# PreibischLab/multiview-simulation

Measured on AMD Instinct MI355X. Metric: simulated Mvoxel/s (views x input voxels / s), 512^3 volume x 8 views, higher is better.
Workload: dtype f32 (f64 attenuation/reductions/Poisson)

## Files before the change

### multiview-simulation_amd/build.py

```python
from __future__ import annotations

import os
import shutil
import subprocess
import sys

HERE = os.path.dirname(os.path.abspath(__file__))
CSRC = os.path.join(HERE, "csrc")
LIB = os.path.join(HERE, "libmvsim.so")
SOURCES = ["api.cpp", "api_view.cpp", "api_host.cpp", "api_sims.cpp", "comm.cpp", "kernels.hip", "extract.hip", "fftconv.hip", "fft_kernels.hip", "rotate_fft.hip", "stencil.hip", "phantom.hip", "beads.hip", "aberrations.hip", "procedural.hip"]
HEADERS = ["common.h", "api_internal.h", "host_pool.h", "jrandom.h", "extract_plan.h", "poisson_dev.h", "fft_dev.h", "../../include/mvsim.h"]
ROCM = os.environ.get("ROCM_PATH", "/opt/rocm")


def _hipcc() -> str:
    for cand in (os.path.join(ROCM, "bin", "hipcc"), shutil.which("hipcc")):
        if cand and os.path.exists(cand):
            return cand
    raise RuntimeError("hipcc not found (ROCm toolchain required to build libmvsim.so)")


def sources():
    return [os.path.join(CSRC, s) for s in SOURCES if os.path.exists(os.path.join(CSRC, s))]


def source_sha() -> str:
    import hashlib
    h = hashlib.sha256()
    files = sorted(sources() + [os.path.normpath(os.path.join(CSRC, x)) for x in HEADERS])
    for f in files:
        h.update(os.path.basename(f).encode() + b"\0")
        with open(f, "rb") as fh:
            h.update(fh.read())
    return h.hexdigest()[:16]


def _common_flags():
    return [
        "--offload-arch=gfx950", "-O3", "-std=c++17", "-fPIC", "-ffp-contract=off", "-fno-fast-math",
        *os.environ.get("MVSIM_EXTRA_CFLAGS", "").split(),
        "-Wall", "-Wno-unused-result", "-I" + os.path.join(ROCM, "include"),
    ]


def is_current() -> bool:
    if not os.path.exists(LIB) or not os.path.exists(LIB + ".flags"):
        return False
    with open(LIB + ".flags") as fh:
        if fh.read() != " ".join(_common_flags()):
            return False
    t = os.path.getmtime(LIB)
    deps = sources() + [os.path.normpath(os.path.join(CSRC, h)) for h in HEADERS] + [os.path.abspath(__file__)]
    return all(os.path.getmtime(d) <= t for d in deps if os.path.exists(d))


def build(force: bool = False, verbose: bool = False) -> str:
    if not force and is_current():
        return LIB
    hipcc = _hipcc()
    objs = []
    os.makedirs(os.path.join(HERE, "build"), exist_ok=True)
    common = _common_flags()
    flags_id = " ".join(common)
    hdr_time = max(os.path.getmtime(os.path.normpath(os.path.join(CSRC, h))) for h in HEADERS)
    hdr_time = max(hdr_time, os.path.getmtime(os.path.abspath(__file__)))
    procs = []
    for src in sources():
        obj = os.path.join(HERE, "build", os.path.basename(src) + ".o")
        objs.append(obj)
        stamp = obj + ".flags"
        fresh = (not force and os.path.exists(obj) and os.path.exists(stamp) and open(stamp).read() == flags_id
                 and os.path.getmtime(obj) >= max(os.path.getmtime(src), hdr_time))
        if fresh:
            continue
        cmd = [hipcc, "-x", "hip", "-c", src, "-o", obj] + common
        if verbose:
            print(" ".join(cmd), file=sys.stderr)
        procs.append((src, stamp, subprocess.Popen(cmd, stdout=subprocess.PIPE, stderr=subprocess.STDOUT, text=True)))
    failed = False
    for src, stamp, p in procs:
        out, _ = p.communicate()
        if p.returncode != 0:
            failed = True
            if os.path.exists(stamp):
                os.remove(stamp)
            sys.stderr.write(f"--- {src} ---\n{out}\n")
        else:
            with open(stamp, "w") as fh:
                fh.write(flags_id)
            if verbose and out.strip():
                sys.stderr.write(out)
    if failed:
        raise RuntimeError("hipcc failed")
    link = [hipcc, "-shared", "-fPIC", "--offload-arch=gfx950", "-o", LIB] + objs + [
# ... 13 lines not shown
```

### multiview-simulation_amd/csrc/api.cpp

```cpp
#include "api_internal.h"

#include <cstdlib>
#include <mutex>
#include <thread>

namespace mvsim {

static thread_local char g_err[512] = "";

void set_error(const char* fmt, ...)
{
    va_list ap;
    va_start(ap, fmt);
    vsnprintf(g_err, sizeof(g_err), fmt, ap);
    va_end(ap);
}

int parse_option(Options& o, const char* name, const char* value)
{
    if (!name || !value) return MVSIM_EINVAL;
    const std::string n(name), v(value);
    auto word = [&](std::initializer_list<std::pair<const char*, int>> words, auto* dst) {
        for (const auto& w : words)
            if (v == w.first) { *dst = w.second; return MVSIM_OK; }
        return MVSIM_EINVAL;
    };
    auto flag = [&](bool* dst) { return word({{"1", 1}, {"on", 1}, {"true", 1}, {"0", 0}, {"off", 0}, {"false", 0}}, dst); };
    auto number = [&](size_t digits, long long lo, long long hi, auto* dst, int when_auto = -1) {
        if (when_auto >= 0 && v == "auto") { *dst = when_auto; return MVSIM_OK; }
        if (v.empty() || v.size() > digits || v.find_first_not_of("0123456789") != std::string::npos) return MVSIM_EINVAL;
        const long long k = atoll(v.c_str());
        if (k < lo || k > hi) return MVSIM_EINVAL;
        *dst = k;
        return MVSIM_OK;
    };
    if (n == "fft_zpass") return word({{"auto", 0}, {"direct", 1}, {"fft", 2}, {"inline", 3}}, &o.zpass);
    if (n == "fft_backend") return word({{"custom", 0}, {"auto", 0}, {"rocfft", 1}}, &o.rocfft);
    if (n == "fused_rotate") return word({{"1", 1}, {"on", 1}, {"lds", 1}, {"0", 0}, {"off", 0}, {"2", 2}, {"lane", 2}, {"3", 3}, {"auto", 3}}, &o.fused_rotate);
    if (n == "poisson_queue") return word({{"1", 1}, {"on", 1}, {"0", 0}, {"off", 0}}, &o.poisson_queue);
    if (n == "poisson_queue_share") return number(2, 1, 16, &o.poisson_queue_share, 0);
    if (n == "attenuate") return word({{"serial", 0}, {"scan", 1}}, &o.attenuate_scan);
    if (n == "early_sum") return flag(&o.early_sum);
    if (n == "zconv_strided") return flag(&o.zconv_strided);
    if (n == "exp") return number(2, 0, 15, &o.exp);
    if (n == "beads_pair_cap") return number(10, 1024, 1LL << 31, &o.beads_pair_cap);
    if (n == "reject_batch") return number(7, 1, 1LL << 20, &o.reject_batch, 0);
    if (n == "fuse_tail") return flag(&o.fuse_tail);
    if (n == "psf_overlap") return flag(&o.psf_overlap);
    if (n == "fused_fftx") return word({{"auto", 2}, {"1", 1}, {"on", 1}, {"0", 0}, {"off", 0}}, &o.fused_fftx);
    if (n == "tail_overlap") return word({{"0", 0}, {"off", 0}, {"1", 1}, {"on", 1}, {"own", 1}, {"2", 2}, {"any", 2}}, &o.tail_overlap);
    if (n == "acq_transfer") return word({{"auto", 1}, {"u16", 1}, {"f32", 0}}, &o.acq_u16);
    if (n == "host_threads") return number(3, 1, 256, &o.host_threads, 0);
    if (n == "view_batch") return word({{"auto", 2}, {"1", 1}, {"on", 1}, {"0", 0}, {"off", 0}}, &o.view_batch);
    if (n == "view_lanes") return number(2, 1, MVSIM_MAX_VIEWS, &o.view_lanes, 0);
    if (n == "graph") { bool g = false; const int rc = flag(&g); o.graph = g ? 1 : 0; return rc; }
    if (n == "broadcast") {
        int how = 0;
        if (word({{"scatter_allgather", 0}, {"auto", 0}, {"ring", 1}, {"peer_copy", 2}, {"pipelined", 3}}, &how) != MVSIM_OK) return MVSIM_EINVAL;
        o.bcast_ring = how == 1; o.bcast_peer_copy = how == 2; o.bcast_pipelined = how == 3;
        return MVSIM_OK;
    }
    if (n == "skip_empty") return flag(&o.skip_empty);
    if (n == "fft_pad") {
        long long a = 0, b = 0, c = 0;
        if (v == "auto" || v.empty()) { o.fft_pad[0] = o.fft_pad[1] = o.fft_pad[2] = 0; return MVSIM_OK; }
        if (sscanf(v.c_str(), "%lld,%lld,%lld", &a, &b, &c) != 3 || a < 0 || b < 0 || c < 0) return MVSIM_EINVAL;
        o.fft_pad[0] = a; o.fft_pad[1] = b; o.fft_pad[2] = c;
        return MVSIM_OK;
    }
    return MVSIM_EINVAL;
}

const Options& env_options()
{
    static Options o;
    static std::once_flag once;
    std::call_once(once, [] {
        if (const char* e = getenv("MVSIM_FFT_ZPASS")) (void)parse_option(o, "fft_zpass", e);
        if (const char* e = getenv("MVSIM_FFT_BACKEND")) (void)parse_option(o, "fft_backend", e);
        if (const char* e = getenv("MVSIM_FFT_PAD")) (void)parse_option(o, "fft_pad", e);
        if (getenv("MVSIM_NO_FUSED_ROTATE")) o.fused_rotate = 0;
        if (getenv("MVSIM_POISSON_NOQUEUE")) o.poisson_queue = 0;
        if (getenv("MVSIM_NO_EARLY_SUM")) o.early_sum = false;
        if (getenv("MVSIM_NO_FUSE_TAIL")) o.fuse_tail = false;
        if (const char* e = getenv("MVSIM_GRAPH")) (void)parse_option(o, "graph", e);
        if (const char* e = getenv("MVSIM_BROADCAST")) (void)parse_option(o, "broadcast", e);
        if (const char* e = getenv("MVSIM_OPTIONS")) {
            std::string all(e);
            size_t pos = 0;
            while (pos < all.size()) {
                size_t end = all.find(';', pos);
                if (end == std::string::npos) end = all.size();
                const std::string kv = all.substr(pos, end - pos);
                const size_t eq = kv.find('=');
                if (eq != std::string::npos) (void)parse_option(o, kv.substr(0, eq).c_str(), kv.substr(eq + 1).c_str());
                pos = end + 1;
            }
        }
    });
    return o;
}

int ensure_lds_attr(mvsim_ctx* ctx, const void* kernel, size_t bytes)
{
    if (bytes <= 64 * 1024) return MVSIM_OK;
    if (bytes > 160 * 1024) { set_error("kernel needs %zu bytes of LDS (> 160 KiB)", bytes); return MVSIM_EINVAL; }
    if (ctx->lds_attr_set.count(kernel)) return MVSIM_OK;
    MVSIM_HIP(hipFuncSetAttribute(kernel, hipFuncAttributeMaxDynamicSharedMemorySize, 160 * 1024));
    ctx->lds_attr_set.insert(kernel);
    return MVSIM_OK;
}

int DevBuf::reserve(size_t need)
{
    if (need <= bytes) return MVSIM_OK;
    if (epoch) *epoch += 1;
    if (p) { (void)hipFree(p); p = nullptr; bytes = 0; }
    hipError_t e = hipMalloc(&p, need);
    if (e != hipSuccess) {
        p = nullptr;
        set_error("hipMalloc(%zu bytes) failed: %s", need, hipGetErrorString(e));
        return MVSIM_ENOMEM;
    }
    bytes = need;
    return MVSIM_OK;
}

void DevBuf::release()
{
    if (p && epoch) *epoch += 1;
    if (p) (void)hipFree(p);
    p = nullptr;
// ... 721 lines not shown
```

### multiview-simulation_amd/csrc/fft_dev.h

```cpp
#pragma once

#include "common.h"

namespace mvsim {
namespace fft {

__device__ __forceinline__ float2 cadd(float2 a, float2 b) { return make_float2(a.x + b.x, a.y + b.y); }
__device__ __forceinline__ float2 csub(float2 a, float2 b) { return make_float2(a.x - b.x, a.y - b.y); }
__device__ __forceinline__ float2 cmul(float2 a, float2 b)
{
    return make_float2(fmaf(a.x, b.x, -a.y * b.y), fmaf(a.x, b.y, a.y * b.x));
}
__device__ __forceinline__ float2 cconj(float2 a) { return make_float2(a.x, -a.y); }
__device__ __forceinline__ float2 mul_mi(float2 a) { return make_float2(a.y, -a.x); }

template <int R> __device__ __forceinline__ void dft(float2* u);

template <> __device__ __forceinline__ void dft<2>(float2* u)
{
    const float2 a = u[0], b = u[1];
    u[0] = cadd(a, b);
    u[1] = csub(a, b);
}

// ... 284 lines not shown
    return -1;
}

struct SrcMap {
    DimMap x, y, z;
    int    enum_y;
};

struct __attribute__((packed, aligned(8))) Pair16 {
    float a, b, c, d;
};

#ifdef MVSIM_DEV_SIZES
#define MVSIM_FFT_SIZES(X) X(280, 7, 5, 8) X(560, 7, 8, 10)
#else
#define MVSIM_FFT_SIZES(X) \
    X(16, 4, 4)            \
    X(18, 9, 2)            \
    X(20, 5, 4)            \
    X(24, 3, 8)            \
    X(32, 4, 8)            \
    X(36, 9, 4)            \
    X(40, 5, 8)            \
    X(48, 3, 4, 4)         \
    X(56, 7, 8)            \
    X(64, 8, 8)            \
    X(72, 9, 8)            \
    X(80, 5, 4, 4)         \
    X(96, 3, 8, 4)         \
    X(112, 7, 4, 4)        \
    X(128, 4, 8, 4)        \
    X(140, 7, 5, 4)        \
    X(144, 9, 4, 4)        \
    X(160, 5, 8, 4)        \
    X(180, 9, 5, 4)        \
    X(192, 3, 8, 8)        \
    X(224, 7, 8, 4)        \
    X(256, 4, 8, 8)        \
    X(280, 7, 5, 8)        \
    X(288, 9, 8, 4)        \
    X(320, 5, 8, 8)        \
    X(350, 7, 10, 5)       \
    X(360, 9, 5, 8)        \
    X(384, 3, 8, 4, 4)     \
    X(448, 7, 8, 8)        \
    X(512, 8, 8, 8)        \
    X(540, 9, 5, 4, 3)     \
    X(560, 7, 8, 10)       \
    X(576, 9, 8, 8)        \
    X(640, 5, 8, 4, 4)     \
    X(720, 9, 8, 10)       \
    X(768, 3, 8, 8, 4)     \
    X(896, 7, 8, 4, 4)     \
    X(1024, 4, 8, 8, 4)    \
    X(1080, 9, 8, 5, 3)    \
    X(1120, 7, 8, 5, 4)    \
    X(1152, 9, 8, 4, 4)    \
    X(1280, 5, 8, 8, 4)    \
    X(1440, 9, 8, 5, 4)    \
    X(1536, 3, 8, 8, 8)    \
    X(1792, 7, 8, 8, 4)    \
    X(2048, 8, 8, 8, 4)    \
    X(2160, 10, 8, 9, 3)   \
    X(2240, 7, 8, 8, 5)
#endif

struct RotFftArgs {
    const float* in;
    float*       rot_out;
    float*       att_out;
    float2*      dst;
    const float2* twg;
    const float2* twx;
    int nx, ny, nz, steps;
    int z_first, nzl;
    int hxp, py;
    int halo_r, halo_l;
    Affine a;
    double delta;
    int*   plane_nz;
};

constexpr bool rot_fftx_len_ok(int len) { return len >= 72 && len <= 576; }
int  launch_rot_fftx(mvsim_ctx* ctx, int M, const RotFftArgs& a, bool write_out);

}
}
```

### multiview-simulation_amd/csrc/fft_kernels.hip

```cpp
#include "common.h"
#include "fft_dev.h"
#include "poisson_dev.h"

#include <algorithm>
#include <cmath>
#include <cstdlib>
#include <cstring>

namespace mvsim {
static int ensure_twiddles(mvsim_ctx* ctx, int L, int kind, const float2** out);
namespace fft {

enum Mode { FWD = 0, INV = 1, CONV = 2, CONVZ = 3 };

struct LinesArgs {
    const float2* src;
    float2*       dst;
    const float2* spec;
    const float2* tw;
    long long     src_es, src_outer, dst_es, dst_outer, spec_es, spec_outer;
    DimMap        lmap;
    int           gap_lo, gap_hi;
    int           outer_skip_lo, outer_skip_len;
    int           store_limit;
// ... 1533 lines not shown

size_t fused_tail_queue_bytes(const int64_t dim[3], const int64_t kdim[3], int inc, bool con_wanted, const Options& opt)
{
    ExtractPlan fp{};
    return fused_tail_geometry(dim, kdim, inc, con_wanted, opt, &fp) ? fp.layout.total_bytes : 0;
}

void custom_fft_release(mvsim_ctx* ctx)
{
    for (auto& kv : ctx->twiddles) (void)hipFree(kv.second);
    ctx->twiddles.clear();
    for (auto& kv : ctx->box_weights) (void)hipFree(kv.second);
    ctx->box_weights.clear();
    ctx->partials_z.release();
    ctx->cfft_f.release();
    ctx->cfft_g.release();
    ctx->cfft_g1.release();
    ctx->cfft_g2.release();
}

bool custom_fft_geometry(const int64_t dim[3], const int64_t kdim[3], int64_t g[5], const Options& opt)
{
    ConvPlan pl;
    if (!conv_plan(dim, kdim, opt, &pl)) return false;
    g[0] = pl.px; g[1] = pl.py; g[2] = pl.zdirect ? pl.n[2] : pl.pz; g[3] = pl.hxp; g[4] = pl.zdirect ? 1 : 0;
    return true;
}

bool custom_fft_batchable(const mvsim_ctx* ctx, const int64_t dim[3], const int64_t kdim[3])
{
    const Options& o = ctx->opt;
    ConvPlan pl;
    return conv_plan(dim, kdim, o, &pl) && pl.early && !o.fuse_tail && o.zpass != 3 && !pl.zinline_auto && pl.ymirror;
}

int rotate_attenuate_fftx(mvsim_ctx* ctx, const float* gt, float* rot_or_null, float* att_or_null, const int64_t dim[3],
                          const int64_t kdim[3], const Affine& inv, double delta, bool* done, const int** plane_nz, int z_first, int nzl)
{
    using namespace fft;
    *done = false;
    if (plane_nz) *plane_nz = nullptr;
    if (ctx->opt.fused_fftx == 0) return MVSIM_OK;
    const bool x_identity = inv.m[0] == 1.0 && inv.m[1] == 0.0 && inv.m[2] == 0.0 && inv.m[3] == 0.0 &&
                            inv.m[4] == 0.0 && inv.m[8] == 0.0;
    if (!x_identity) return MVSIM_OK;
    ConvPlan pl;
    if (!conv_plan(dim, kdim, ctx->opt, &pl)) return MVSIM_OK;
    const int nx = pl.n[0], ny = pl.n[1], nz = pl.n[2], kx = pl.k[0];
    if (nzl < 0) { z_first = 0; nzl = nz; }
    if (z_first < 0 || nzl < 1 || z_first + nzl > nz) return MVSIM_OK;
    if (!pl.ymirror || nx > 1024 || nx < 64 || kx > nx || nx > ny) return MVSIM_OK;
    const int px = pl.px, py = pl.py, M = pl.M, hxp = pl.hxp;
    if (!rot_fftx_len_ok(M)) return MVSIM_OK;
    if (ctx->opt.fused_fftx == 2 && (int64_t)nx * nzl < 131072) return MVSIM_OK;
    const size_t cbytes = pl.spectrum_bytes(nzl, 0, 0, 1);
    MVSIM_TRY(ctx->cfft_f.reserve(cbytes));
    MVSIM_TRY(ctx->cfft_g.reserve(cbytes));
    const float2 *tw_m, *tw_px;
    MVSIM_TRY(ensure_twiddles(ctx, M, 0, &tw_m));
    MVSIM_TRY(ensure_twiddles(ctx, px, 1, &tw_px));
    RotFftArgs a{};
    a.in = gt; a.rot_out = rot_or_null; a.att_out = att_or_null; a.dst = ctx->cfft_f.as<float2>();
    a.twg = tw_m; a.twx = tw_px;
    a.nx = nx; a.ny = ny; a.nz = nz; a.steps = nx;
    a.z_first = z_first; a.nzl = nzl;
    a.hxp = hxp; a.py = py;
    a.halo_r = kx / 2; a.halo_l = kx - 1 - kx / 2;
    a.a = inv; a.delta = delta;
    bool want_flags = plane_nz && ctx->opt.skip_empty && nzl == nz;
    if (want_flags) {
        if (!ctx->empty_hint) {
            MVSIM_HIP(hipHostMalloc(reinterpret_cast<void**>(&ctx->empty_hint), 4 * sizeof(int), hipHostMallocDefault));
            ctx->empty_hint[0] = -1; ctx->empty_hint[1] = -1; ctx->empty_hint[2] = 0; ctx->empty_hint[3] = 0;
        }
        const int hint = *reinterpret_cast<volatile int*>(ctx->empty_hint);
        if (hint == 0 && ctx->views_since_flags < 15) { want_flags = false; ctx->views_since_flags += 1; }
        else ctx->views_since_flags = 0;
    }
    if (want_flags) {
        MVSIM_TRY(ctx->plane_flags.reserve((size_t)(3 * nz + 1024) * sizeof(int)));
        a.plane_nz = ctx->plane_flags.as<int>();
        *plane_nz = a.plane_nz;
    }
    MVSIM_TRY(launch_rot_fftx(ctx, M, a, rot_or_null != nullptr || att_or_null != nullptr));
    *done = true;
    return MVSIM_OK;
}

namespace fft {
struct ConvRun {
    const ConvPlan& pl;
    SlabRange slab;
    const LenEntry* xlen;
    bool is_slab;
    long long plane;
    int V, zstride;
    int nzp;
    int nk;
    int zs_chunk, zs_frows;
    size_t zs_lds;
    bool zinline;
    long long corr_n;
    float corr_min, corr_target;
    const float2 *tw_m, *tw_px, *tw_py, *tw_pz;
    float2 *F, *G, *G1, *G2;
    double* scal;
    const int *pnz, *pnz_dil;
    const unsigned int* pnz_bits;
};

static int psf_passes(mvsim_ctx* ctx, const ConvRun& r, const float* psf)
{
    const ConvPlan& pl = r.pl;
    const int kx = pl.k[0], ky = pl.k[1], kz = pl.k[2], hxp = pl.hxp, V = r.V;
    SrcMap m{};
    m.x = DimMap{kx, pl.px, kx - kx / 2, kx / 2, 1, kx / 2};
    m.y = DimMap{ky, ky, ky, 0, 1, 0};
    m.z = DimMap{kz * V, kz * V, kz * V, 0, 1, 0};
    MVSIM_TRY(r.xlen->r2c(ctx, psf, m, r.G1, r.tw_m, r.tw_px, hxp, (long long)ky * kz * V));
    LinesArgs a{};
    a.src = r.G1; a.dst = r.G2; a.spec = nullptr; a.tw = r.tw_py;
    a.src_es = hxp; a.src_outer = (long long)hxp * ky;
    a.dst_es = hxp; a.dst_outer = r.plane;
    if (pl.zdirect) { a.dst_outer = (long long)ZB * hxp; a.dst_blk = (long long)kz * V * ZB * hxp; }
    a.lmap = DimMap{ky, pl.py, ky - ky / 2, ky / 2, 1, ky / 2};
    MVSIM_TRY(launch_lines(ctx, pl.py, FWD, true, a, hxp / pl.tile_y, kz * V));
    if (pl.zdirect) return MVSIM_OK;
    LinesArgs c{};
    c.src = r.G2; c.dst = r.G; c.spec = nullptr; c.tw = r.tw_pz;
    c.src_es = r.plane; c.src_outer = hxp;
    c.dst_es = r.plane; c.dst_outer = hxp;
    c.lmap = DimMap{kz, pl.pz, kz - kz / 2, kz / 2, 1, kz / 2};
    c.dst_tile_major = 1;
    return launch_lines(ctx, pl.pz, FWD, true, c, hxp / pl.tile_z, pl.py);
}

static int psf_spectrum(mvsim_ctx* ctx, const ConvRun& r, const float* psf)
{
    hipStream_t s = ctx->stream;
    const bool side = ctx->opt.psf_overlap && (int64_t)r.pl.n[0] * r.pl.n[1] * r.pl.n[2] >= (int64_t)1 << 24;
    ctx->psf_on_side = side;
    if (side) {
        if (!ctx->side_stream) {
            MVSIM_HIP(hipStreamCreateWithFlags(&ctx->side_stream, hipStreamNonBlocking));
            MVSIM_HIP(hipEventCreateWithFlags(&ctx->ev_fork, hipEventDisableTiming));
            MVSIM_HIP(hipEventCreateWithFlags(&ctx->ev_join, hipEventDisableTiming));
        }
        MVSIM_HIP(hipEventRecord(ctx->ev_fork, s));
        MVSIM_HIP(hipStreamWaitEvent(ctx->side_stream, ctx->ev_fork, 0));
        ctx->stream = ctx->side_stream;
    }
    ev_begin(ctx, ST_PSF);
    const int rc = psf_passes(ctx, r, psf);
    ev_end(ctx, ST_PSF);
    if (side) {
        ctx->stream = s;
        MVSIM_HIP(hipEventRecord(ctx->ev_join, ctx->side_stream));
    }
    return rc;
}

static int pass_a(mvsim_ctx* ctx, const ConvRun& r, const float* img)
{
    const ConvPlan& pl = r.pl;
    const int planes = r.slab.nz_in * r.V;
    SrcMap m{};
    DimMap* dm[3] = {&m.x, &m.y, &m.z};
// ... 288 lines not shown
```

### multiview-simulation_amd/csrc/rotate_fft.hip

```cpp
#include "common.h"
#include "fft_dev.h"

#include <type_traits>

namespace mvsim {
namespace fft {

struct __attribute__((aligned(16))) RowGeoF {
    double    w00, w10, w11, w01;
    long long off00;
    int       kind;
    int       pad;
};
constexpr int geo_chunk_f(int G) { return G == 1 ? 512 : 128; }
constexpr int UF = 8;
#ifndef MVSIM_ROTFFT_PREFETCH
#define MVSIM_ROTFFT_PREFETCH 0
#endif

template <class PLAN, bool WRITE_OUT, int G>
__global__ __launch_bounds__(1024) void k_rotate_attenuate_fftx(RotFftArgs p)
{
    constexpr int M = PLAN::len, LP = M + 1, U = UF, GEO_CHUNK_F = geo_chunk_f(G);
    extern __shared__ __align__(16) float2 lds[];
    float2* rowbuf = lds;
    float2* tw = lds + 2 * G * U * LP;
    float2* twx_l = tw + M + (M & 1);
    RowGeoF* geo = reinterpret_cast<RowGeoF*>(twx_l + (M + 1) + ((M + 1) & 1));
    int* bclass = reinterpret_cast<int*>(geo + GEO_CHUNK_F);
    unsigned int* wmask = reinterpret_cast<unsigned int*>(bclass + GEO_CHUNK_F / U);
    const int nx = p.nx, ny = p.ny, nz = p.nz, steps = p.steps;
    const int x = threadIdx.x;
    const int lane = x & 63, wave = __builtin_amdgcn_readfirstlane(x >> 6), nwaves = (int)blockDim.x >> 6;
    const int slab = (gridDim.x + 7) / 8;
    const int hs = slab / 2, jb = (int)(blockIdx.x / 8u), kb = (int)(blockIdx.x % 8u);
    const int zl = (hs > 0 && slab == 2 * hs) ? ((jb < hs) ? kb * hs + jb : (int)gridDim.x / 2 + kb * hs + (jb - hs))
                                              : kb * slab + jb;
    if (zl >= p.nzl) return;
    const int z = p.z_first + zl;
    const bool active = x < nx;
    const long long row = (long long)nx;
    const long long plane = row * ny;
    const long long out_plane = plane * zl;
    const double l2 = (double)z;
    const char* __restrict__ in_b = reinterpret_cast<const char*>(p.in);
    const long long row_b = row * 4, plane_b = plane * 4;
    const unsigned xoff = (unsigned)(active ? x : nx - 1) * 4u;
    const Affine& a = p.a;
    const double delta = p.delta;
    const int Px = 2 * M;
    const int pos_r = (active && x >= nx - 1 - p.halo_r && x <= nx - 2) ? 2 * nx - 2 - x : -1;
    const int pos_l = (active && x >= 1 && x <= p.halo_l) ? Px - x : -1;
    const int gap_lo = nx + p.halo_r, gap_len = Px - p.halo_l - gap_lo;
    for (int i = x; i < M; i += (int)blockDim.x) tw[i] = p.twg[i];
    for (int i = x; i <= M; i += (int)blockDim.x) twx_l[i] = p.twx[i];

    auto transform_store = [&](float2* wbuf, int y) {
        PLAN::template run<1>(wbuf, tw, lane);
        float2* __restrict__ drow = p.dst + ((long long)zl * p.py + y) * p.hxp;
        constexpr int HQ = M / 4;
#pragma unroll 1
        for (int q = lane; q < HQ; q += 64) {
            float2 lo[2], hi[2];
#pragma unroll
            for (int h = 0; h < 2; ++h) {
                const int k = 2 * q + h;
                const float2 zk = wbuf[k];
                const float2 zm = cconj(wbuf[k == 0 ? 0 : M - k]);
                const float2 sm = cadd(zk, zm), d = csub(zk, zm);
                const float2 wd = cmul(twx_l[k], d);
                const float2 t = make_float2(wd.y, -wd.x);
                lo[h] = cadd(sm, t);
                hi[h] = cconj(csub(sm, t));
            }
            *reinterpret_cast<float4*>(drow + 2 * q) = make_float4(lo[0].x, lo[0].y, lo[1].x, lo[1].y);
            *reinterpret_cast<Pair16*>(drow + M - 2 * q - 1) = Pair16{hi[1].x, hi[1].y, hi[0].x, hi[0].y};
        }
        const int nmid = M - 4 * HQ + 1;
        const int ntail = nmid + (p.hxp - M - 1);
        for (int u = lane; u < ntail; u += 64) {
            if (u < nmid) {
                const int k = 2 * HQ + u;
                const float2 zk = wbuf[k == M ? 0 : k];
                const float2 zm = cconj(wbuf[k == 0 ? 0 : M - k]);
// ... 159 lines not shown
                            const float a10 = (active && t10) ? p00[row + x] : 0.f;
                            const float a11 = (active && t11) ? p00[row + plane + x] : 0.f;
                            const float a01 = (active && t01) ? p00[plane + x] : 0.f;
                            r = (float)((double)a00 * g->w00);
                            r += (float)((double)a10 * g->w10);
                            r += (float)((double)a11 * g->w11);
                            r += (float)((double)a01 * g->w01);
                            const double d = (double)r;
                            n = fmax(n - d * delta * n, 0.0);
                            val[u] = (float)(d * n);
                        }
                        if (WRITE_OUT && active) {
                            if (p.rot_out) p.rot_out[o + x] = r;
                            if (p.att_out) p.att_out[o + x] = val[u];
                        }
                    }
                }
            }
            {
                unsigned int rowmask = 0u;
#pragma unroll
                for (int u = 0; u < U; ++u)
                    if (__builtin_amdgcn_ballot_w64(active && (__float_as_uint(val[u]) << 1) != 0u) != 0ull) rowmask |= 1u << u;
                if (lane == 0) wmask[(buf * G + fill) * 16 + wave] = rowmask;
                plane_any |= rowmask;
            }
            float* __restrict__ rb = reinterpret_cast<float*>(rowbuf + ((size_t)buf * G + fill) * U * LP);
            ysub[fill] = y0;
            nsub[fill] = nrows;
            fill += 1;
#pragma unroll
            for (int u = 0; u < U; ++u) {
                float* __restrict__ rr = rb + (size_t)u * 2 * LP;
                if (active) rr[x] = val[u];
                if (pos_r >= 0) rr[pos_r] = val[u];
                if (pos_l >= 0) rr[pos_l] = val[u];
                for (int gpos = x; gpos < gap_len; gpos += (int)blockDim.x) rr[gap_lo + gpos] = 0.f;
            }
            have_pref = r0 + U < cnt && __builtin_amdgcn_readfirstlane(bclass[r0 / U + 1]) == 1;
            if (have_pref) issue_loads(r0 + U, std::integral_constant<int, 0>{}, std::integral_constant<int, UPRE>{});
            if (fill == G) flush_round();
        }
        if (fill > 0) flush_round();
    }
    if (p.plane_nz) {
        unsigned int* blk_any = wmask + 2 * G * 16;
        __syncthreads();
        if (x == 0) *blk_any = 0u;
        __syncthreads();
        if (lane == 0 && plane_any != 0u) atomicOr(blk_any, 1u);
        __syncthreads();
        if (x == 0) p.plane_nz[zl] = (int)*blk_any;
    }
    for (int yy = ny - 1 - steps; yy >= 0; --yy) {
        if (WRITE_OUT && active) {
            if (p.att_out) p.att_out[out_plane + (long long)yy * row + x] = 0.f;
            if (p.rot_out) {
                const double l1 = (double)yy;
                const double py = 0.0 * a.m[4] + l1 * a.m[5] + l2 * a.m[6] + a.m[7];
                const double pz = 0.0 * a.m[8] + l1 * a.m[9] + l2 * a.m[10] + a.m[11];
                const double fy = floor(py), fz = floor(pz);
                float o = 0.f;
                if (fy >= -1.0 && fz >= -1.0 && fy < (double)ny && fz < (double)nz) {
                    const int sy = (int)fy, sz = (int)fz;
                    const double w1 = py - fy, w2 = pz - fz;
                    const double w1n = 1.0 - w1, w2n = 1.0 - w2;
                    const double q00 = 1.0 * w1n * w2n, q10 = 1.0 * w1 * w2n, q11 = 1.0 * w1 * w2, q01 = 1.0 * w1n * w2;
                    const bool ya = sy >= 0, yb = sy + 1 < ny, za = sz >= 0, zb = sz + 1 < nz;
                    const float* __restrict__ pin = p.in + x;
                    const float a00 = (ya && za) ? pin[row * (sy + (long long)ny * sz)] : 0.f;
                    const float a10 = (yb && za) ? pin[row * (sy + 1 + (long long)ny * sz)] : 0.f;
                    const float a11 = (yb && zb) ? pin[row * (sy + 1 + (long long)ny * (sz + 1))] : 0.f;
                    const float a01 = (ya && zb) ? pin[row * (sy + (long long)ny * (sz + 1))] : 0.f;
                    o = (float)((double)a00 * q00); o += (float)((double)a10 * q10);
                    o += (float)((double)a11 * q11); o += (float)((double)a01 * q01);
                }
                p.rot_out[out_plane + (long long)yy * row + x] = o;
            }
        }
        if ((ny - 1 - steps - yy) % nwaves == wave) zero_row(yy);
    }
}

template <class PLAN>
static int launch_rot_fftx_t(mvsim_ctx* ctx, const RotFftArgs& a, bool write_out)
{
    constexpr int M = PLAN::len;
    const int waves = (a.nx + 63) / 64;
    const int G = waves > 8 ? 2 : 1;
    const size_t lds = (size_t)(2 * G * UF * (M + 1) + M + (M & 1) + (M + 1) + ((M + 1) & 1)) * sizeof(float2) + (size_t)geo_chunk_f(G) * sizeof(RowGeoF) +
                       (size_t)(geo_chunk_f(G) / UF) * sizeof(int) + (size_t)(2 * G * 16 + 4) * sizeof(unsigned int);
    if (lds > 160 * 1024) { set_error("fused rotate + x transform: %zu bytes of LDS", lds); return MVSIM_EINVAL; }
    dim3 grid((unsigned)((a.nzl + 7) / 8 * 8)), block((unsigned)(waves * 64));
#define MVSIM_RF(W_, G_)                                                                                            \
    do {                                                                                                            \
        MVSIM_TRY(ensure_lds_attr(ctx, reinterpret_cast<const void*>(k_rotate_attenuate_fftx<PLAN, W_, G_>), lds)); \
        hipLaunchKernelGGL((k_rotate_attenuate_fftx<PLAN, W_, G_>), grid, block, lds, ctx->stream, a);              \
    } while (0)
    if constexpr (M >= 280) {
        if (G == 2) {
            if (write_out) MVSIM_RF(true, 2); else MVSIM_RF(false, 2);
            MVSIM_HIP(hipGetLastError());
            return MVSIM_OK;
        }
    }
    if (G == 2) { set_error("fused rotate + x transform: no 16-wave instance for half length %d", M); return MVSIM_EINVAL; }
    if (write_out) MVSIM_RF(true, 1); else MVSIM_RF(false, 1);
#undef MVSIM_RF
    MVSIM_HIP(hipGetLastError());
    return MVSIM_OK;
}

template <int LL, int... Rs>
static int launch_rot_fftx_pick(mvsim_ctx* ctx, const RotFftArgs& a, bool write_out)
{
    if constexpr (rot_fftx_len_ok(LL)) return launch_rot_fftx_t<Plan<LL, Rs...>>(ctx, a, write_out);
    set_error("fused rotate + x transform: half length %d is not instantiated", LL);
    return MVSIM_EINVAL;
}

int launch_rot_fftx(mvsim_ctx* ctx, int M, const RotFftArgs& a, bool write_out)
{
    switch (M) {
#define X(LL, ...) case LL: return launch_rot_fftx_pick<LL, __VA_ARGS__>(ctx, a, write_out);
        MVSIM_FFT_SIZES(X)
#undef X
    }
    set_error("fused rotate + x transform: no plan for half length %d", M);
    return MVSIM_EINVAL;
}

}
}
```

Measured before the change: 77150.

## Add wave-specialized rotate+attenuate+x-FFT kernel with walker and transformer roles

Adds a variant of the fused rotate/attenuate/x-transform kernel in which each block is split into walker waves and a few extra transformer waves. Walkers gather the rotated rows, attenuate them and fill double-buffered LDS row rounds. Transformer waves run at raised priority and do the FFT and post-processing on the previous round, synchronised by one barrier per round. The aim is to overlap the memory-bound gather with the FFT compute instead of running them back to back. It is selected under the default 'auto' setting for small enough sizes, at the cost of larger blocks, more registers and LDS pressure, and a new round scheduler header.

```diff
diff --git a/multiview-simulation_amd/build.py b/multiview-simulation_amd/build.py
--- a/multiview-simulation_amd/build.py
+++ b/multiview-simulation_amd/build.py
@@ -9,7 +9,7 @@
 CSRC = os.path.join(HERE, "csrc")
 LIB = os.path.join(HERE, "libmvsim.so")
 SOURCES = ["api.cpp", "api_view.cpp", "api_host.cpp", "api_sims.cpp", "comm.cpp", "kernels.hip", "extract.hip", "fftconv.hip", "fft_kernels.hip", "rotate_fft.hip", "stencil.hip", "phantom.hip", "beads.hip", "aberrations.hip", "procedural.hip"]
-HEADERS = ["common.h", "api_internal.h", "host_pool.h", "jrandom.h", "extract_plan.h", "poisson_dev.h", "fft_dev.h", "../../include/mvsim.h"]
+HEADERS = ["common.h", "api_internal.h", "host_pool.h", "jrandom.h", "extract_plan.h", "poisson_dev.h", "fft_dev.h", "rotate_rounds.h", "../../include/mvsim.h"]
 ROCM = os.environ.get("ROCM_PATH", "/opt/rocm")
 
 
diff --git a/multiview-simulation_amd/csrc/api.cpp b/multiview-simulation_amd/csrc/api.cpp
--- a/multiview-simulation_amd/csrc/api.cpp
+++ b/multiview-simulation_amd/csrc/api.cpp
@@ -47,7 +47,7 @@
     if (n == "reject_batch") return number(7, 1, 1LL << 20, &o.reject_batch, 0);
     if (n == "fuse_tail") return flag(&o.fuse_tail);
     if (n == "psf_overlap") return flag(&o.psf_overlap);
-    if (n == "fused_fftx") return word({{"auto", 2}, {"1", 1}, {"on", 1}, {"0", 0}, {"off", 0}}, &o.fused_fftx);
+    if (n == "fused_fftx") return word({{"auto", 2}, {"1", 1}, {"on", 1}, {"0", 0}, {"off", 0}, {"roles", 3}}, &o.fused_fftx);
     if (n == "tail_overlap") return word({{"0", 0}, {"off", 0}, {"1", 1}, {"on", 1}, {"own", 1}, {"2", 2}, {"any", 2}}, &o.tail_overlap);
     if (n == "acq_transfer") return word({{"auto", 1}, {"u16", 1}, {"f32", 0}}, &o.acq_u16);
     if (n == "host_threads") return number(3, 1, 256, &o.host_threads, 0);
diff --git a/multiview-simulation_amd/csrc/fft_dev.h b/multiview-simulation_amd/csrc/fft_dev.h
--- a/multiview-simulation_amd/csrc/fft_dev.h
+++ b/multiview-simulation_amd/csrc/fft_dev.h
@@ -390,7 +390,7 @@
 };
 
 constexpr bool rot_fftx_len_ok(int len) { return len >= 72 && len <= 576; }
-int  launch_rot_fftx(mvsim_ctx* ctx, int M, const RotFftArgs& a, bool write_out);
-
-}
-}
+int  launch_rot_fftx(mvsim_ctx* ctx, int M, const RotFftArgs& a, bool write_out, bool roles);
+
+}
+}
diff --git a/multiview-simulation_amd/csrc/fft_kernels.hip b/multiview-simulation_amd/csrc/fft_kernels.hip
--- a/multiview-simulation_amd/csrc/fft_kernels.hip
+++ b/multiview-simulation_amd/csrc/fft_kernels.hip
@@ -1639,7 +1639,7 @@
         a.plane_nz = ctx->plane_flags.as<int>();
         *plane_nz = a.plane_nz;
     }
-    MVSIM_TRY(launch_rot_fftx(ctx, M, a, rot_or_null != nullptr || att_or_null != nullptr));
+    MVSIM_TRY(launch_rot_fftx(ctx, M, a, rot_or_null != nullptr || att_or_null != nullptr, ctx->opt.fused_fftx >= 2));
     *done = true;
     return MVSIM_OK;
 }
diff --git a/multiview-simulation_amd/csrc/rotate_fft.hip b/multiview-simulation_amd/csrc/rotate_fft.hip
--- a/multiview-simulation_amd/csrc/rotate_fft.hip
+++ b/multiview-simulation_amd/csrc/rotate_fft.hip
@@ -1,5 +1,6 @@
 #include "common.h"
 #include "fft_dev.h"
+#include "rotate_rounds.h"
 
 #include <type_traits>
 
@@ -325,12 +326,339 @@
     }
 }
 
+#ifndef MVSIM_ROTFFT_ROLE_WAVES
+#define MVSIM_ROTFFT_ROLE_WAVES 4
+#endif
+constexpr int ROLE_T = MVSIM_ROTFFT_ROLE_WAVES;
+static_assert(ROLE_T == 2 || ROLE_T == 4, "transformer waves per block");
+static_assert(UF == ROT_ROUND_ROWS && UF % ROLE_T == 0, "round geometry");
+constexpr bool rot_fftx_roles_len_ok(int len) { return rot_fftx_len_ok(len) && len <= 288; }
+
+template <int M>
+__device__ __forceinline__ void rot_post_store(const float2* wbuf, const float2* twx_l, float2* __restrict__ drow, int hxp, int lane)
+{
+    constexpr int HQ = M / 4;
+#pragma unroll 1
+    for (int q = lane; q < HQ; q += 64) {
+        float2 lo[2], hi[2];
+#pragma unroll
+        for (int h = 0; h < 2; ++h) {
+            const int k = 2 * q + h;
+            const float2 zk = wbuf[k];
+            const float2 zm = cconj(wbuf[k == 0 ? 0 : M - k]);
+            const float2 sm = cadd(zk, zm), d = csub(zk, zm);
+            const float2 wd = cmul(twx_l[k], d);
+            const float2 t = make_float2(wd.y, -wd.x);
+            lo[h] = cadd(sm, t);
+            hi[h] = cconj(csub(sm, t));
+        }
+        *reinterpret_cast<float4*>(drow + 2 * q) = make_float4(lo[0].x, lo[0].y, lo[1].x, lo[1].y);
+        *reinterpret_cast<Pair16*>(drow + M - 2 * q - 1) = Pair16{hi[1].x, hi[1].y, hi[0].x, hi[0].y};
+    }
+    const int nmid = M - 4 * HQ + 1;
+    const int ntail = nmid + (hxp - M - 1);
+    for (int u = lane; u < ntail; u += 64) {
+        if (u < nmid) {
+            const int k = 2 * HQ + u;
+            const float2 zk = wbuf[k == M ? 0 : k];
+            const float2 zm = cconj(wbuf[k == 0 ? 0 : M - k]);
+            const float2 sm = cadd(zk, zm), d = csub(zk, zm);
+            const float2 wd = cmul(twx_l[k], d);
+            drow[k] = cadd(sm, make_float2(wd.y, -wd.x));
+        } else {
+            drow[M + 1 + (u - nmid)] = make_float2(0.f, 0.f);
+        }
+    }
+}
+
+template <class PLAN, bool WRITE_OUT, int T>
+__global__ __launch_bounds__((8 + T) * 64, (8 + T) / 2) void k_rotate_attenuate_fftx_roles(RotFftArgs p)
+{
+    constexpr int M = PLAN::len, LP = M + 1, U = UF, GEO_CHUNK_F = geo_chunk_f(1), RW = rot_round_group(T);
+    extern __shared__ __align__(16) float2 lds[];
+    float2* rowbuf = lds;
+    float2* tw = lds + 2 * U * LP;
+    float2* twx_l = tw + M + (M & 1);
+    RowGeoF* geo = reinterpret_cast<RowGeoF*>(twx_l + (M + 1) + ((M + 1) & 1));
+    int* bclass = reinterpret_cast<int*>(geo + GEO_CHUNK_F);
+    unsigned int* wmask = reinterpret_cast<unsigned int*>(bclass + GEO_CHUNK_F / U);
+    const int nx = p.nx, ny = p.ny, nz = p.nz, steps = p.steps;
+    const int x = threadIdx.x;
+    const int lane = x & 63, wave = __builtin_amdgcn_readfirstlane(x >> 6);
+    const int nwalk = ((int)blockDim.x >> 6) - T, walk_threads = nwalk * 64;
+    const bool walker = wave < nwalk;
+    const int tr = wave - nwalk;
+    const int slab = (gridDim.x + 7) / 8;
+    const int hs = slab / 2, jb = (int)(blockIdx.x / 8u), kb = (int)(blockIdx.x % 8u);
+    const int zl = (hs > 0 && slab == 2 * hs) ? ((jb < hs) ? kb * hs + jb : (int)gridDim.x / 2 + kb * hs + (jb - hs))
+                                              : kb * slab + jb;
+    if (zl >= p.nzl) return;
+    const int z = p.z_first + zl;
+    const bool active = x < nx;
+    const long long row = (long long)nx;
+    const long long plane = row * ny;
+    const long long out_plane = plane * zl;
+    const double l2 = (double)z;
+    const char* __restrict__ in_b = reinterpret_cast<const char*>(p.in);
+    const unsigned xoff = (unsigned)(active ? x : nx - 1) * 4u;
+    const unsigned o10 = xoff + (unsigned)(row * 4), o01 = xoff + (unsigned)(plane * 4), o11 = o10 + (unsigned)(plane * 4);
+    const Affine& a = p.a;
+    const double delta = p.delta;
+    const int Px = 2 * M;
+    const int pos_r = (active && x >= nx - 1 - p.halo_r && x <= nx - 2) ? 2 * nx - 2 - x : -1;
+    const int pos_l = (active && x >= 1 && x <= p.halo_l) ? Px - x : -1;
+    const int gap_lo = nx + p.halo_r, gap_len = Px - p.halo_l - gap_lo;
+    for (int i = x; i < M; i += (int)blockDim.x) tw[i] = p.twg[i];
+    for (int i = x; i <= M; i += (int)blockDim.x) twx_l[i] = p.twx[i];
+
+    auto zero_row = [&](int y) {
+        float4* __restrict__ drow = reinterpret_cast<float4*>(p.dst + ((long long)zl * p.py + y) * p.hxp);
+        for (int i = lane; i < p.hxp / 2; i += 64) drow[i] = make_float4(0.f, 0.f, 0.f, 0.f);
+    };
+    auto round_barrier = [&]() { asm volatile("s_waitcnt lgkmcnt(0)\n\ts_barrier" ::: "memory"); };
+    auto cls_of = [&](int b) { return __builtin_amdgcn_readfirstlane(bclass[b]); };
+
+    double n = 1.0;
+    unsigned int plane_any = 0u;
+    const int cnt = steps;
+    __syncthreads();
+    for (int r = x; r < cnt; r += (int)blockDim.x) {
+        const int yy = ny - 1 - r;
+        const double l1 = (double)yy;
+        const double py = 0.0 * a.m[4] + l1 * a.m[5] + l2 * a.m[6] + a.m[7];
+        const double pz = 0.0 * a.m[8] + l1 * a.m[9] + l2 * a.m[10] + a.m[11];
+        const double fy = floor(py), fz = floor(pz);
+        RowGeoF g;
+        g.w00 = g.w10 = g.w11 = g.w01 = 0.0;
+        g.off00 = 0;
+        g.kind = 0;
+        g.pad = 0;
+        if (fy >= -1.0 && fz >= -1.0 && fy < (double)ny && fz < (double)nz) {
+            const int sy = (int)fy, sz = (int)fz;
+            const double w1 = py - fy, w2 = pz - fz;
+            const double w1n = 1.0 - w1, w2n = 1.0 - w2;
+            g.w00 = 1.0 * w1n * w2n; g.w10 = 1.0 * w1 * w2n; g.w11 = 1.0 * w1 * w2; g.w01 = 1.0 * w1n * w2;
+            const bool ya = sy >= 0, yb = sy + 1 < ny, za = sz >= 0, zb = sz + 1 < nz;
+            g.off00 = row * (sy + (long long)ny * sz) * 4;
+            const int m = ((ya && za) ? 1 : 0) | ((yb && za) ? 2 : 0) | ((yb && zb) ? 4 : 0) | ((ya && zb) ? 8 : 0);
+            g.kind = m == 15 ? 1 : (m == 0 ? 0 : (2 | (m << 8)));
+        }
+        geo[r] = g;
+    }
+    __syncthreads();
+    for (int bq = x; bq < (cnt + U - 1) / U; bq += (int)blockDim.x) {
+        bool all1 = true, all0 = true;
+        for (int u = 0; u < U; ++u) {
+            const int r = bq * U + u;
+            if (r < cnt) {
+                const int k = geo[r].kind;
+                all1 = all1 && k == 1;
+                all0 = all0 && k == 0;
+            } else {
+                all1 = false;
+                all0 = false;
+            }
+        }
+        bclass[bq] = all1 ? 1 : (all0 ? 0 : 2);
+    }
+    __syncthreads();
+    RotRounds rounds = rot_rounds_begin(cnt, 0);
+    RotBatch b;
+    if (!walker) {
+        __builtin_amdgcn_s_setprio(1);
+        while (rot_rounds_next(rounds, cls_of, b)) {
+            const int y0 = ny - 1 - b.r0;
+            if (b.cls == 0) {
+                for (int j = tr; j < U; j += T) zero_row(y0 - j);
+                continue;
+            }
+            round_barrier();
+            unsigned int any = 0u;
+            for (int w = 0; w < nwalk; ++w) any |= wmask[b.buf * 16 + w];
+#ifdef MVSIM_EXP_ROTFFT_NOFFT
+            any = 0u;
+#endif
+            any = __builtin_amdgcn_readfirstlane(any);
+#pragma unroll 1
+            for (int u = tr * RW; u < (tr + 1) * RW && u < b.nrows; ++u) {
+                const int y = y0 - u;
+                if ((any >> u) & 1u) {
+                    float2* wbuf = rowbuf + ((size_t)b.buf * U + u) * LP;
+                    PLAN::template run<1>(wbuf, tw, lane);
+                    rot_post_store<M>(wbuf, twx_l, p.dst + ((long long)zl * p.py + y) * p.hxp, p.hxp, lane);
+                } else {
+                    zero_row(y);
+                }
+            }
+        }
+    } else {
+        while (rot_rounds_next(rounds, cls_of, b)) {
+            const int r0 = b.r0, y0 = ny - 1 - r0, nrows = b.nrows;
+            if (b.cls == 0) {
+                if (WRITE_OUT && active) {
+#pragma unroll
+                    for (int u = 0; u < U; ++u) {
+                        const long long o = out_plane + (long long)(y0 - u) * row;
+                        if (p.rot_out) p.rot_out[o + x] = 0.f;
+                        if (p.att_out) p.att_out[o + x] = 0.f;
+                    }
+                }
+                continue;
+            }
+            float val[U];
+            if (b.cls == 1) {
+                float pv00[U], pv10[U], pv11[U], pv01[U];
+                auto issue_row = [&](int u) {
+                    const long long off = geo[r0 + u].off00;
+                    const unsigned lo = __builtin_amdgcn_readfirstlane((unsigned)(unsigned long long)off);
+                    const unsigned hi = __builtin_amdgcn_readfirstlane((unsigned)((unsigned long long)off >> 32));
+                    const char* __restrict__ p00 = in_b + (long long)(((unsigned long long)hi << 32) | lo);
+                    pv00[u] = *reinterpret_cast<const float*>(p00 + xoff);
+                    pv10[u] = *reinterpret_cast<const float*>(p00 + o10);
+                    pv11[u] = *reinterpret_cast<const float*>(p00 + o11);
+                    pv01[u] = *reinterpret_cast<const float*>(p00 + o01);
+                };
+#pragma unroll
+                for (int u = 0; u < U; ++u) issue_row(u);
+#pragma unroll
+                for (int u = 0; u < U; ++u) {
+                    const unsigned bits = __float_as_uint(pv00[u]) | __float_as_uint(pv10[u]) | __float_as_uint(pv11[u]) | __float_as_uint(pv01[u]);
+                    if (__builtin_amdgcn_ballot_w64((bits << 1) != 0u) == 0ull) {
+                        val[u] = 0.f;
+                        if (WRITE_OUT && active) {
+                            const long long ob = (out_plane + (long long)(y0 - u) * row) * 4;
+                            if (p.rot_out) *reinterpret_cast<float*>(reinterpret_cast<char*>(p.rot_out) + ob + xoff) = 0.f;
+                            if (p.att_out) *reinterpret_cast<float*>(reinterpret_cast<char*>(p.att_out) + ob + xoff) = 0.f;
+                        }
+                        continue;
+                    }
+                    const RowGeoF* g = &geo[r0 + u];
+                    float r = (float)((double)pv00[u] * g->w00);
+                    r += (float)((double)pv10[u] * g->w10);
+                    r += (float)((double)pv11[u] * g->w11);
+                    r += (float)((double)pv01[u] * g->w01);
+                    const double d = (double)r;
+                    n = fmax(n - d * delta * n, 0.0);
+                    val[u] = (float)(d * n);
+                    if (WRITE_OUT && active) {
+                        const long long ob = (out_plane + (long long)(y0 - u) * row) * 4;
+                        if (p.rot_out) *reinterpret_cast<float*>(reinterpret_cast<char*>(p.rot_out) + ob + xoff) = r;
+                        if (p.att_out) *reinterpret_cast<float*>(reinterpret_cast<char*>(p.att_out) + ob + xoff) = val[u];
+                    }
+                }
+            } else {
+#pragma unroll
+                for (int u = 0; u < U; ++u) {
+                    val[u] = 0.f;
+                    if (u < nrows) {
+                        const RowGeoF* g = &geo[r0 + u];
+                        const int kind = __builtin_amdgcn_readfirstlane(g->kind);
+                        const long long o = out_plane + (long long)(y0 - u) * row;
+                        float r = 0.f;
+                        if (kind != 0) {
+                            const float* __restrict__ p00 = reinterpret_cast<const float*>(in_b + g->off00);
+                            const bool t00 = kind == 1 || (kind & (1 << 8)), t10 = kind == 1 || (kind & (2 << 8));
+                            const bool t11 = kind == 1 || (kind & (4 << 8)), t01 = kind == 1 || (kind & (8 << 8));
+                            const float a00 = (active && t00) ? p00[x] : 0.f;
+                            const float a10 = (active && t10) ? p00[row + x] : 0.f;
+                            const float a11 = (active && t11) ? p00[row + plane + x] : 0.f;
+                            const float a01 = (active && t01) ? p00[plane + x] : 0.f;
+                            r = (float)((double)a00 * g->w00);
+                            r += (float)((double)a10 * g->w10);
+                            r += (float)((double)a11 * g->w11);
+                            r += (float)((double)a01 * g->w01);
+                            const double d = (double)r;
+                            n = fmax(n - d * delta * n, 0.0);
+                            val[u] = (float)(d * n);
+                        }
+                        if (WRITE_OUT && active) {
+                            if (p.rot_out) p.rot_out[o + x] = r;
+                            if (p.att_out) p.att_out[o + x] = val[u];
+                        }
+                    }
+                }
+            }
+            {
+                unsigned int rowmask = 0u;
+#pragma unroll
+                for (int u = 0; u < U; ++u)
+                    if (__builtin_amdgcn_ballot_w64(active && (__float_as_uint(val[u]) << 1) != 0u) != 0ull) rowmask |= 1u << u;
+                if (lane == 0) wmask[b.buf * 16 + wave] = rowmask;
+                plane_any |= rowmask;
+            }
+            float* __restrict__ rb = reinterpret_cast<float*>(rowbuf + (size_t)b.buf * U * LP);
+#pragma unroll
+            for (int u = 0; u < U; ++u) {
+                float* __restrict__ rr = rb + (size_t)u * 2 * LP;
+                if (active) rr[x] = val[u];
+                if (pos_r >= 0) rr[pos_r] = val[u];
+                if (pos_l >= 0) rr[pos_l] = val[u];
+                for (int gpos = x; gpos < gap_len; gpos += walk_threads) rr[gap_lo + gpos] = 0.f;
+            }
+            round_barrier();
+        }
+    }
+    if (p.plane_nz) {
+        unsigned int* blk_any = wmask + 2 * 16;
+        __syncthreads();
+        if (x == 0) *blk_any = 0u;
+        __syncthreads();
+        if (lane == 0 && plane_any != 0u) atomicOr(blk_any, 1u);
+        __syncthreads();
+        if (x == 0) p.plane_nz[zl] = (int)*blk_any;
+    }
+    for (int yy = ny - 1 - steps; yy >= 0; --yy) {
+        if (WRITE_OUT && active) {
+            if (p.att_out) p.att_out[out_plane + (long long)yy * row + x] = 0.f;
+            if (p.rot_out) {
+                const double l1 = (double)yy;
+                const double py = 0.0 * a.m[4] + l1 * a.m[5] + l2 * a.m[6] + a.m[7];
+                const double pz = 0.0 * a.m[8] + l1 * a.m[9] + l2 * a.m[10] + a.m[11];
+                const double fy = floor(py), fz = floor(pz);
+                float o = 0.f;
+                if (fy >= -1.0 && fz >= -1.0 && fy < (double)ny && fz < (double)nz) {
+                    const int sy = (int)fy, sz = (int)fz;
+                    const double w1 = py - fy, w2 = pz - fz;
+                    const double w1n = 1.0 - w1, w2n = 1.0 - w2;
+                    const double q00 = 1.0 * w1n * w2n, q10 = 1.0 * w1 * w2n, q11 = 1.0 * w1 * w2, q01 = 1.0 * w1n * w2;
+                    const bool ya = sy >= 0, yb = sy + 1 < ny, za = sz >= 0, zb = sz + 1 < nz;
+                    const float* __restrict__ pin = p.in + x;
+                    const float a00 = (ya && za) ? pin[row * (sy + (long long)ny * sz)] : 0.f;
+                    const float a10 = (yb && za) ? pin[row * (sy + 1 + (long long)ny * sz)] : 0.f;
+                    const float a11 = (yb && zb) ? pin[row * (sy + 1 + (long long)ny * (sz + 1))] : 0.f;
+                    const float a01 = (ya && zb) ? pin[row * (sy + (long long)ny * (sz + 1))] : 0.f;
+                    o = (float)((double)a00 * q00); o += (float)((double)a10 * q10);
+                    o += (float)((double)a11 * q11); o += (float)((double)a01 * q01);
+                }
+                p.rot_out[out_plane + (long long)yy * row + x] = o;
+            }
+        }
+        if (!walker && (ny - 1 - steps - yy) % T == tr) zero_row(yy);
+    }
+}
+
 template <class PLAN>
-static int launch_rot_fftx_t(mvsim_ctx* ctx, const RotFftArgs& a, bool write_out)
+static int launch_rot_fftx_t(mvsim_ctx* ctx, const RotFftArgs& a, bool write_out, bool roles)
 {
     constexpr int M = PLAN::len;
     const int waves = (a.nx + 63) / 64;
     const int G = waves > 8 ? 2 : 1;
+    if constexpr (rot_fftx_roles_len_ok(M)) {
+        if (roles && waves <= 8 && a.steps <= geo_chunk_f(1) && ((int64_t)a.nx * a.ny + 2 * (int64_t)a.nx) * 4 < (int64_t)1 << 32) {
+            const size_t lds = (size_t)(2 * UF * (M + 1) + M + (M & 1) + (M + 1) + ((M + 1) & 1)) * sizeof(float2) + (size_t)geo_chunk_f(1) * sizeof(RowGeoF) +
+                               (size_t)(geo_chunk_f(1) / UF) * sizeof(int) + (size_t)(2 * 16 + 4) * sizeof(unsigned int);
+            dim3 grid((unsigned)((a.nzl + 7) / 8 * 8)), block((unsigned)((waves + ROLE_T) * 64));
+            if (write_out) {
+                MVSIM_TRY(ensure_lds_attr(ctx, reinterpret_cast<const void*>(k_rotate_attenuate_fftx_roles<PLAN, true, ROLE_T>), lds));
+                hipLaunchKernelGGL((k_rotate_attenuate_fftx_roles<PLAN, true, ROLE_T>), grid, block, lds, ctx->stream, a);
+            } else {
+                MVSIM_TRY(ensure_lds_attr(ctx, reinterpret_cast<const void*>(k_rotate_attenuate_fftx_roles<PLAN, false, ROLE_T>), lds));
+                hipLaunchKernelGGL((k_rotate_attenuate_fftx_roles<PLAN, false, ROLE_T>), grid, block, lds, ctx->stream, a);
+            }
+            MVSIM_HIP(hipGetLastError());
+            return MVSIM_OK;
+        }
+    }
     const size_t lds = (size_t)(2 * G * UF * (M + 1) + M + (M & 1) + (M + 1) + ((M + 1) & 1)) * sizeof(float2) + (size_t)geo_chunk_f(G) * sizeof(RowGeoF) +
                        (size_t)(geo_chunk_f(G) / UF) * sizeof(int) + (size_t)(2 * G * 16 + 4) * sizeof(unsigned int);
     if (lds > 160 * 1024) { set_error("fused rotate + x transform: %zu bytes of LDS", lds); return MVSIM_EINVAL; }
@@ -355,17 +683,17 @@
 }
 
 template <int LL, int... Rs>
-static int launch_rot_fftx_pick(mvsim_ctx* ctx, const RotFftArgs& a, bool write_out)
+static int launch_rot_fftx_pick(mvsim_ctx* ctx, const RotFftArgs& a, bool write_out, bool roles)
 {
-    if constexpr (rot_fftx_len_ok(LL)) return launch_rot_fftx_t<Plan<LL, Rs...>>(ctx, a, write_out);
+    if constexpr (rot_fftx_len_ok(LL)) return launch_rot_fftx_t<Plan<LL, Rs...>>(ctx, a, write_out, roles);
     set_error("fused rotate + x transform: half length %d is not instantiated", LL);
     return MVSIM_EINVAL;
 }
 
-int launch_rot_fftx(mvsim_ctx* ctx, int M, const RotFftArgs& a, bool write_out)
+int launch_rot_fftx(mvsim_ctx* ctx, int M, const RotFftArgs& a, bool write_out, bool roles)
 {
     switch (M) {
-#define X(LL, ...) case LL: return launch_rot_fftx_pick<LL, __VA_ARGS__>(ctx, a, write_out);
+#define X(LL, ...) case LL: return launch_rot_fftx_pick<LL, __VA_ARGS__>(ctx, a, write_out, roles);
         MVSIM_FFT_SIZES(X)
 #undef X
     }
diff --git a/multiview-simulation_amd/csrc/rotate_rounds.h b/multiview-simulation_amd/csrc/rotate_rounds.h
--- /dev/null
+++ b/multiview-simulation_amd/csrc/rotate_rounds.h
@@ -0,0 +1,54 @@
+#pragma once
+
+#if defined(__HIPCC__)
+#define MVSIM_RR_FN __host__ __device__
+#else
+#define MVSIM_RR_FN
+#endif
+
+namespace mvsim {
+namespace fft {
+
+constexpr int ROT_ROUND_ROWS = 8;
+constexpr int ROT_ROUND_BUFS = 2;
+
+struct RotRounds {
+    int cnt;
+    int r0;
+    int buf;
+};
+
+struct RotBatch {
+    int r0;
+    int nrows;
+    int cls;
+    int buf;
+};
+
+MVSIM_RR_FN inline RotRounds rot_rounds_begin(int cnt, int buf)
+{
+    return RotRounds{cnt, 0, buf};
+}
+
+template <class CLS>
+MVSIM_RR_FN inline bool rot_rounds_next(RotRounds& st, const CLS& cls_of, RotBatch& b)
+{
+    if (st.r0 >= st.cnt) return false;
+    b.r0 = st.r0;
+    b.nrows = st.cnt - st.r0 < ROT_ROUND_ROWS ? st.cnt - st.r0 : ROT_ROUND_ROWS;
+    b.cls = cls_of(st.r0 / ROT_ROUND_ROWS);
+    if (b.cls == 0) {
+        b.buf = -1;
+    } else {
+        b.buf = st.buf;
+        st.buf = (st.buf + 1) % ROT_ROUND_BUFS;
+    }
+    st.r0 += ROT_ROUND_ROWS;
+    return true;
+}
+
+MVSIM_RR_FN constexpr int rot_round_group(int nt) { return ROT_ROUND_ROWS / nt; }
+MVSIM_RR_FN constexpr int rot_round_owner(int u, int nt) { return u / rot_round_group(nt); }
+
+}
+}
```

Result: faster. 79180, median of 6 (+2.6%).
